# zoharl3/mantaflow

Measured on AMD Instinct MI355X. Metric: Mcells/s per step (advect+CG+FLIP), 256^3 grid, higher is better.
Workload: dtype f32; 1 GPU; 256^3 smoke step on 1 x MI355X: advectSemiLagrange(density, order 2) + advectSemiLagrange(vel, order 2) + setWallBcs + solvePressure (MIC-CG, cgAccuracy 1e-3); parallelism=single GPU

## Files before the change

### mantaflow_amd/csrc/pressure.hip

```cpp
#include "common.h"
#include "pressure.h"
#include <float.h>
#include <stdlib.h>
#include <stdio.h>
#include <type_traits>

using namespace mf;

static thread_local int g_last_shortcut[3] = {0, 0, 0};


__device__ __forceinline__ float wave_shr1(float v) {
	return __int_as_float(__builtin_amdgcn_update_dpp(__float_as_int(v), __float_as_int(v), 0x138, 0xf, 0xf, false));
}
__device__ __forceinline__ float wave_shl1(float v) {
	return __int_as_float(__builtin_amdgcn_update_dpp(__float_as_int(v), __float_as_int(v), 0x130, 0xf, 0xf, false));
}
__device__ __forceinline__ int4 unpack_flags(unsigned w) {
	return make_int4((w & 0x1u) ? MF_FLUID : 0, (w & 0x100u) ? MF_FLUID : 0, (w & 0x10000u) ? MF_FLUID : 0, (w & 0x1000000u) ? MF_FLUID : 0);
}
template <unsigned BIT>
__device__ __forceinline__ float4 unpack_coef(unsigned w) {
	return make_float4((w & BIT) ? -1.f : 0.f, (w & (BIT << 8)) ? -1.f : 0.f, (w & (BIT << 16)) ? -1.f : 0.f, (w & (BIT << 24)) ? -1.f : 0.f);
}
#ifndef AM_NT
#define AM_NT 2
#endif
#ifndef PCG_NT_MI
#define PCG_NT_MI 10
#endif
constexpr int64_t PCG_NT_CELLS = (int64_t)PCG_NT_MI << 20;
#ifndef AMP_NT
#define AMP_NT 1
#endif
template <bool DOT, bool IS3D, int R, bool PACKED>
__global__ void __launch_bounds__(BLOCK)
k_apply_matrix_v5(Dim d, const int32_t* __restrict__ flags, float* __restrict__ dst, const float* __restrict__ src,
                  const float* __restrict__ A0, const float* __restrict__ Ai, const float* __restrict__ Aj,
                  const float* __restrict__ Ak, double* __restrict__ partials, const CgScalars* __restrict__ sc, int jgroups, int tpb,
                  const unsigned char* __restrict__ pack, int dk0, int dk1, int a0p, const int* __restrict__ bempty = nullptr, int nbj = 0,
                  const int* __restrict__ outside_bad = nullptr, const int* __restrict__ xr = nullptr) {
	if (DOT && sc->done) return;
	const int qx = d.sx >> 2;
	const int64_t nthr = (int64_t)qx * jgroups * d.sz;
	const int vb0 = xcd_swizzle(blockIdx.x, gridDim.x) * tpb;
	double acc = 0.0;
#pragma unroll 1
	for (int t = 0; t < tpb; t++) {
	const int64_t T0 = (int64_t)(vb0 + t) * BLOCK + threadIdx.x;
	const bool live = T0 < nthr;
	const int64_t T = live ? T0 : nthr - 1;
	const int qi = (int)(T % qx);
	const int64_t rg = T / qx;
	const int j0 = (int)(rg % jgroups) * R;
	const int k = (int)(rg / jgroups);
	int q_lo = 0, q_hi = qx;
	if (IS3D && bempty && outside_bad[0] == 0) {
		if (xr) {
			q_lo = (xr[0] & ~7) >> 2;
			q_hi = ((xr[1] + 7) & ~7) >> 2;
		}
		if (bempty[(k >> 3) * nbj + (j0 >> 3)] || qi < q_lo || qi >= q_hi) continue;
	}
	const int lane = threadIdx.x & 63;
	const float4 z4 = make_float4(0.f, 0.f, 0.f, 0.f);
	const int64_t Y = d.Y, Z = d.Z;
	const int64_t row0 = ((int64_t)k * d.sy + j0) * d.sx + 4 * qi;
	int4 f[R];
	float4 sv[R + 2], ajv[R + 1], a0[R], ai[R], ak[R], akm[R], szm[R], szp[R];
	float sl[R], al[R], sr[R];
	{
		const int jm = (rg > 0) ? -1 : 0;
		sv[0] = *(const float4*)(src + row0 + jm * Y);
		if (PACKED) ajv[0] = unpack_coef<4u>(*(const unsigned*)(pack + row0 + jm * Y));
		else ajv[0] = *(const float4*)(Aj + row0 + jm * Y);
	}
#pragma unroll
	for (int r = 0; r < R; r++) {
		const int jr = (j0 + r < d.sy) ? r : (d.sy - 1 - j0);
		const int64_t idx = row0 + jr * Y;
		sv[r + 1] = ((AMP_NT & 1) && (!DOT || (a0p & 2))) ? ld_nt4(src + idx) : *(const float4*)(src + idx);
		unsigned pw = 0;
		if (PACKED) pw = *(const unsigned*)(pack + idx);
		if (PACKED && (a0p & 1)) a0[r] = make_float4((float)((pw >> 4) & 15u), (float)((pw >> 12) & 15u), (float)((pw >> 20) & 15u), (float)((pw >> 28) & 15u));
		else a0[r] = (AM_NT >= 1) ? ld_nt4(A0 + idx) : *(const float4*)(A0 + idx);
		if (PACKED) {
			f[r] = unpack_flags(pw);
			ajv[r + 1] = unpack_coef<4u>(pw);
			ai[r] = unpack_coef<2u>(pw);
		} else {
			f[r] = (AM_NT >= 1) ? ld_nt4i(flags + idx) : *(const int4*)(flags + idx);
			ajv[r + 1] = (AM_NT >= 3) ? ld_nt4(Aj + idx) : *(const float4*)(Aj + idx);
			ai[r] = (AM_NT >= 1) ? ld_nt4(Ai + idx) : *(const float4*)(Ai + idx);
		}
		if (IS3D) {
			const int64_t im = (k > 0) ? idx - Z : idx, ip = (k < d.sz - 1) ? idx + Z : idx;
			if (PACKED) {
				ak[r] = unpack_coef<8u>(pw);
				akm[r] = unpack_coef<8u>(*(const unsigned*)(pack + im));
			} else {
				ak[r] = (AM_NT >= 3) ? ld_nt4(Ak + idx) : *(const float4*)(Ak + idx);
				akm[r] = *(const float4*)(Ak + im);
			}
			szm[r] = (AMP_NT & 2) ? ld_nt4(src + im) : *(const float4*)(src + im);
			szp[r] = (AMP_NT & 2) ? ld_nt4(src + ip) : *(const float4*)(src + ip);
		}
	}
	{
		const int jr = (j0 + R < d.sy) ? R : (d.sy - j0 - ((k < d.sz - 1) ? 0 : 1));
		sv[R + 1] = *(const float4*)(src + row0 + jr * Y);
	}
	const bool edge_l = (lane == 0) || (qi == 0) || (qi == q_lo), edge_r = (lane == 63) || (qi == qx - 1) || (qi == q_hi - 1);
#pragma unroll
	for (int r = 0; r < R; r++) {
		const int jr = (j0 + r < d.sy) ? r : (d.sy - 1 - j0);
		const int64_t idx = row0 + jr * Y;
		sl[r] = wave_shr1(sv[r + 1].w);
		al[r] = wave_shr1(ai[r].w);
		sr[r] = wave_shl1(sv[r + 1].x);
		if (edge_l) {
			sl[r] = (idx > 0) ? src[idx - 1] : 0.f;
			if (PACKED) al[r] = (idx > 0 && (pack[idx - 1] & 2u)) ? -1.f : 0.f;
			else al[r] = (idx > 0) ? Ai[idx - 1] : 0.f;
		}
		if (edge_r) sr[r] = (idx + 4 < d.n) ? src[idx + 4] : 0.f;
	}
#pragma unroll
	for (int r = 0; r < R; r++) {
		const int j = j0 + r;
		if (j >= d.sy) break;
		const int4 fl = f[r];
		const float4 s = sv[r + 1];
		float4 res = s;
		if ((fl.x | fl.y | fl.z | fl.w) & MF_FLUID) {
			const float4 sym = (j > 0 || k > 0) ? sv[r] : z4, ajm = (j > 0 || k > 0) ? ajv[r] : z4;
			const float4 syp = (j < d.sy - 1) ? sv[r + 2] : (k < d.sz - 1) ? sv[R + 1] : z4, aj = ajv[r + 1];
			float4 zm = z4, am = z4, zp = z4, akc = z4;
			if (IS3D) {
				akc = ak[r];
				if (k > 0) {
					zm = szm[r];
					am = akm[r];
				}
				if (k < d.sz - 1) zp = szp[r];
			}
#define CELL5(c, SL, AL, SR)                                                                      \
	if (fl.c & MF_FLUID) {                                                                        \
		float v = s.c * a0[r].c;                                                                  \
		v = v + (SL) * (AL);                                                                      \
		v = v + (SR) * ai[r].c;                                                                   \
		v = v + sym.c * ajm.c;                                                                    \
		v = v + syp.c * aj.c;                                                                     \
		if (IS3D) {                                                                               \
			v = v + zm.c * am.c;                                                                  \
			v = v + zp.c * akc.c;                                                                 \
		}                                                                                         \
		res.c = v;                                                                                \
	}
			CELL5(x, sl[r], al[r], s.y)
			CELL5(y, s.x, ai[r].x, s.z)
			CELL5(z, s.y, ai[r].y, s.w)
			CELL5(w, s.z, ai[r].z, sr[r])
#undef CELL5
		}
		if (live) {
			if (AM_NT >= 2 && (!DOT || (a0p & 2))) st_nt4(dst + row0 + r * Y, res);
			else *(float4*)(dst + row0 + r * Y) = res;
			if (DOT && k >= dk0 && k < dk1) {
				const float p0 = res.x * s.x, p1 = res.y * s.y, p2 = res.z * s.z, p3 = res.w * s.w;
				acc += (double)p0;
				acc += (double)p1;
				acc += (double)p2;
				acc += (double)p3;
			}
		}
	}
	}
	if (DOT) {
		acc = block_sum(acc);
		if (threadIdx.x == 0) partials[blockIdx.x] = acc;
	}
}

template <bool DOT>
__global__ void __launch_bounds__(BLOCK)
k_apply_matrix_scalar(Dim d, const int32_t* __restrict__ flags, float* __restrict__ dst, const float* __restrict__ src,
                      const float* __restrict__ A0, const float* __restrict__ Ai, const float* __restrict__ Aj,
                      const float* __restrict__ Ak, double* __restrict__ partials, const CgScalars* __restrict__ sc) {
	if (DOT && sc->done) return;
	double acc = 0.0;
	for (int64_t idx = blockIdx.x * (int64_t)BLOCK + threadIdx.x; idx < d.n; idx += (int64_t)gridDim.x * BLOCK) {
		const float s = src[idx];
		float v = s;
		if (flags[idx] & MF_FLUID) {
			const int64_t Y = d.Y, Z = d.Z;
			v = s * A0[idx];
			v = v + ((idx >= 1) ? src[idx - 1] * Ai[idx - 1] : 0.f);
			v = v + ((idx + 1 < d.n) ? src[idx + 1] : 0.f) * Ai[idx];
			v = v + ((idx >= Y) ? src[idx - Y] * Aj[idx - Y] : 0.f);
			v = v + ((idx + Y < d.n) ? src[idx + Y] : 0.f) * Aj[idx];
			if (d.is3d) {
				v = v + ((idx >= Z) ? src[idx - Z] * Ak[idx - Z] : 0.f);
				v = v + ((idx + Z < d.n) ? src[idx + Z] : 0.f) * Ak[idx];
			}
		}
		dst[idx] = v;
		if (DOT) {
			const float p = v * s;
			acc += (double)p;
		}
	}
	if (DOT) {
		acc = block_sum(acc);
		if (threadIdx.x == 0) partials[blockIdx.x] = acc;
	}
}


struct AmOpts {
	const unsigned char* pack = nullptr;
	bool a0p = false;
	int dk0 = 0, dk1 = 0x7fffffff;
	const int* bempty = nullptr;
	int nbj = 0;
	const int* outside_bad = nullptr;
	const int* xr = nullptr;
	int nt = -1;
};
template <bool DOT>
static int launch_apply_matrix(const Dim& d, const int32_t* flags, float* dst, const float* src, const float* A0,
                               const float* Ai, const float* Aj, const float* Ak, double* partials,
                               const CgScalars* sc, hipStream_t st, const AmOpts& o = AmOpts{}, int* nblocks = nullptr, bool* ranged = nullptr) {
	if (ranged) *ranged = false;
	const int a0pn = (o.a0p ? 1 : 0) | ((DOT && (o.nt < 0 ? d.n > PCG_NT_CELLS : o.nt != 0)) ? 2 : 0);
	const bool vec = (d.sx % 4 == 0) && al16(flags) && al16(dst) && al16(src) && al16(A0) && al16(Ai) && al16(Aj) && al16(Ak);
	int nb;
	if (vec) {
		constexpr int R = 2;
		const int jgroups = (d.sy + R - 1) / R;
		const int64_t vblocks = ((int64_t)(d.sx >> 2) * jgroups * d.sz + BLOCK - 1) / BLOCK;
		const int tpb = (int)((vblocks + MAX_BLOCKS - 1) / MAX_BLOCKS);
		nb = (int)((vblocks + tpb - 1) / tpb);
		auto kern = !d.is3d ? k_apply_matrix_v5<DOT, false, R, false> : o.pack ? k_apply_matrix_v5<DOT, true, R, true> : k_apply_matrix_v5<DOT, true, R, false>;
		hipLaunchKernelGGL(kern, dim3(nb), dim3(BLOCK), 0, st, d, flags, dst, src, A0, Ai, Aj, Ak, partials, sc, jgroups, tpb, o.pack, o.dk0, o.dk1, a0pn,
		                   o.bempty, o.nbj, o.outside_bad, o.xr);
		if (ranged) *ranged = true;
	} else {
		nb = blocks_for(d.n, BLOCK, 2048);
		hipLaunchKernelGGL((k_apply_matrix_scalar<DOT>), dim3(nb), dim3(BLOCK), 0, st, d, flags, dst, src, A0, Ai, Aj, Ak, partials, sc);
	}
	MF_LAUNCH_CHECK();
	if (nblocks) *nblocks = nb;
	return 0;
}

__global__ void __launch_bounds__(BLOCK)
k_make_laplace(Dim d, const int32_t* __restrict__ flags, float* __restrict__ A0, float* __restrict__ Ai,
               float* __restrict__ Aj, float* __restrict__ Ak, const float* __restrict__ fr) {
	CELL_IJK(d)
	if (!INTERIOR(d)) return;
	if (!(flags[idx] & MF_FLUID)) return;
	const int64_t Y = d.Y, Z = d.Z;
	float a0 = A0[idx];
	if (!fr) {
		if (!(flags[idx - 1] & MF_OBSTACLE)) a0 = (float)((double)a0 + 1.);
		if (!(flags[idx + 1] & MF_OBSTACLE)) a0 = (float)((double)a0 + 1.);
		if (!(flags[idx - Y] & MF_OBSTACLE)) a0 = (float)((double)a0 + 1.);
		if (!(flags[idx + Y] & MF_OBSTACLE)) a0 = (float)((double)a0 + 1.);
		if (d.is3d && !(flags[idx - Z] & MF_OBSTACLE)) a0 = (float)((double)a0 + 1.);
		if (d.is3d && !(flags[idx + Z] & MF_OBSTACLE)) a0 = (float)((double)a0 + 1.);
		if (flags[idx + 1] & MF_FLUID) Ai[idx] = -1.f;
		if (flags[idx + Y] & MF_FLUID) Aj[idx] = -1.f;
		if (d.is3d && (flags[idx + Z] & MF_FLUID)) Ak[idx] = -1.f;
	} else {
		const float *fx = fr, *fy = fr + d.n, *fz = fr + 2 * d.n;
		a0 += fx[idx];
		a0 += fx[idx + 1];
		a0 += fy[idx];
		a0 += fy[idx + Y];
		if (d.is3d) a0 += fz[idx];
		if (d.is3d) a0 += fz[idx + Z];
		if (flags[idx + 1] & MF_FLUID) Ai[idx] = -fx[idx + 1];
		if (flags[idx + Y] & MF_FLUID) Aj[idx] = -fy[idx + Y];
		if (d.is3d && (flags[idx + Z] & MF_FLUID)) Ak[idx] = -fz[idx + Z];
	}
	A0[idx] = a0;
}

__device__ __forceinline__ float thetaHelper(float inside, float outside) {
	const float denom = inside - outside;
	if ((double)denom > -1e-04) return 0.5f;
	const float q = inside / denom;
	const float m = q < 1.f ? q : 1.f;
	return 0.f < m ? m : 0.f;
}
__device__ __forceinline__ float ghostFluidHelper(int64_t idx, int64_t offset, const float* __restrict__ phi, float gfClamp) {
	const float alpha = thetaHelper(phi[idx], phi[idx + offset]);
	if (alpha < gfClamp) return gfClamp;
	return (float)(1. - (1. / (double)alpha));
}
__device__ __forceinline__ float surfTensHelper(int64_t idx, int64_t offset, const float* __restrict__ phi,
                                                const float* __restrict__ curv, float surfTens, float gfClamp) {
	return surfTens * (curv[idx + offset] - ghostFluidHelper(idx, offset, phi, gfClamp) * curv[idx]);
}
__device__ __forceinline__ bool ghostFluidWasClamped(int64_t idx, int64_t offset, const float* __restrict__ phi, float gfClamp) {
	return thetaHelper(phi[idx], phi[idx + offset]) < gfClamp;
}

__global__ void __launch_bounds__(BLOCK)
k_make_rhs(Dim d, const int32_t* __restrict__ flags, float* __restrict__ rhs, const float* __restrict__ vel,
           const float* __restrict__ pcc, const float* __restrict__ fr, const float* __restrict__ ob,
           const float* __restrict__ phi, const float* __restrict__ curv, float surfTens, float gfClamp,
           double* __restrict__ partials) {
	double mysum = 0.0, mycnt = 0.0;
	const int64_t X = 1, Y = d.Y, Z = d.Z, n = d.n;
	const float *vx = vel, *vy = vel + n, *vz = vel + 2 * n;
	for (int64_t idx = blockIdx.x * (int64_t)BLOCK + threadIdx.x; idx < n; idx += (int64_t)gridDim.x * BLOCK) {
		const int i = (int)(idx % d.sx);
		const int j = (int)((idx / d.sx) % d.sy);
		const int k = (int)(idx / ((int64_t)d.sx * d.sy));
		if (!INTERIOR(d)) continue;
		if (!(flags[idx] & MF_FLUID)) {
			rhs[idx] = 0.f;
			continue;
		}
		float set;
		if (!fr) {
			set = vx[idx] - vx[idx + X] + vy[idx] - vy[idx + Y];
			if (d.is3d) set += vz[idx] - vz[idx + Z];
		} else {
			const float *fx = fr, *fy = fr + n, *fz = fr + 2 * n;
			set = fx[idx] * vx[idx] - fx[idx + X] * vx[idx + X] + fy[idx] * vy[idx] - fy[idx + Y] * vy[idx + Y];
			if (d.is3d) set += fz[idx] * vz[idx] - fz[idx + Z] * vz[idx + Z];
			if (ob) {
				const float *ox = ob, *oy = ob + n, *oz = ob + 2 * n;
				set += (1 - fx[idx]) * ox[idx] - (1 - fx[idx + X]) * ox[idx + X] + (1 - fy[idx]) * oy[idx] -
				       (1 - fy[idx + Y]) * oy[idx + Y];
				if (d.is3d) set += (1 - fz[idx]) * oz[idx] - (1 - fz[idx + Z]) * oz[idx + Z];
			}
		}
		if (phi && curv) {
			if (flags[idx - X] & MF_EMPTY) set += surfTensHelper(idx, -X, phi, curv, surfTens, gfClamp);
			if (flags[idx + X] & MF_EMPTY) set += surfTensHelper(idx, +X, phi, curv, surfTens, gfClamp);
			if (flags[idx - Y] & MF_EMPTY) set += surfTensHelper(idx, -Y, phi, curv, surfTens, gfClamp);
			if (flags[idx + Y] & MF_EMPTY) set += surfTensHelper(idx, +Y, phi, curv, surfTens, gfClamp);
			if (d.is3d) {
				if (flags[idx - Z] & MF_EMPTY) set += surfTensHelper(idx, -Z, phi, curv, surfTens, gfClamp);
				if (flags[idx + Z] & MF_EMPTY) set += surfTensHelper(idx, +Z, phi, curv, surfTens, gfClamp);
			}
		}
		if (pcc) set += pcc[idx];
		mysum += (double)set;
		mycnt += 1.0;
		rhs[idx] = set;
	}
	mysum = block_sum(mysum);
	__syncthreads();
	mycnt = block_sum(mycnt);
	if (threadIdx.x == 0) {
		partials[blockIdx.x] = mysum;
		partials[MAX_BLOCKS + blockIdx.x] = mycnt;
	}
}
__global__ void __launch_bounds__(BLOCK) k_sum2_finish(int nb, const double* __restrict__ p0, const double* __restrict__ p1, double* __restrict__ out) {
	double a = strided_sum(p0, nb), b = strided_sum(p1, nb);
	a = block_sum(a);
	__syncthreads();
	b = block_sum(b);
	if (threadIdx.x == 0) {
		out[0] = a;
		out[1] = b;
	}
}

__global__ void __launch_bounds__(BLOCK)
k_ghost_fluid_diag(Dim d, float* __restrict__ A0, const int32_t* __restrict__ flags, const float* __restrict__ phi, float gfClamp) {
	CELL_IJK(d)
	if (!INTERIOR(d)) return;
	if (!(flags[idx] & MF_FLUID)) return;
	const int64_t X = 1, Y = d.Y, Z = d.Z;
	float a = A0[idx];
	if (flags[idx - X] & MF_EMPTY) a -= ghostFluidHelper(idx, -X, phi, gfClamp);
	if (flags[idx + X] & MF_EMPTY) a -= ghostFluidHelper(idx, +X, phi, gfClamp);
	if (flags[idx - Y] & MF_EMPTY) a -= ghostFluidHelper(idx, -Y, phi, gfClamp);
	if (flags[idx + Y] & MF_EMPTY) a -= ghostFluidHelper(idx, +Y, phi, gfClamp);
	if (d.is3d) {
		if (flags[idx - Z] & MF_EMPTY) a -= ghostFluidHelper(idx, -Z, phi, gfClamp);
		if (flags[idx + Z] & MF_EMPTY) a -= ghostFluidHelper(idx, +Z, phi, gfClamp);
	}
	A0[idx] = a;
}

__global__ void __launch_bounds__(BLOCK)
k_correct_velocity(Dim d, const int32_t* __restrict__ flags, float* __restrict__ vel, const float* __restrict__ p) {
	CELL_IJK(d)
	if (!INTERIOR(d)) return;
	const int64_t X = 1, Y = d.Y, Z = d.Z, n = d.n;
	float *vx = vel, *vy = vel + n, *vz = vel + 2 * n;
	const int f = flags[idx];
	if (f & MF_FLUID) {
		const float pc = p[idx];
		float x = vx[idx], y = vy[idx], z = d.is3d ? vz[idx] : 0.f;
		const int fxm = flags[idx - X], fym = flags[idx - Y], fzm = d.is3d ? flags[idx - Z] : 0;
		if (fxm & MF_FLUID) x -= (pc - p[idx - X]);
		if (fym & MF_FLUID) y -= (pc - p[idx - Y]);
		if (d.is3d && (fzm & MF_FLUID)) z -= (pc - p[idx - Z]);
		if (fxm & MF_EMPTY) x -= pc;
		if (fym & MF_EMPTY) y -= pc;
		if (d.is3d && (fzm & MF_EMPTY)) z -= pc;
		vx[idx] = x;
		vy[idx] = y;
		if (d.is3d) vz[idx] = z;
	} else if ((f & MF_EMPTY) && !(f & MF_OUTFLOW)) {
		if (flags[idx - X] & MF_FLUID) vx[idx] += p[idx - X]; else vx[idx] = 0.f;
		if (flags[idx - Y] & MF_FLUID) vy[idx] += p[idx - Y]; else vy[idx] = 0.f;
		if (d.is3d) {
			if (flags[idx - Z] & MF_FLUID) vz[idx] += p[idx - Z]; else vz[idx] = 0.f;
		}
	}
}

__global__ void __launch_bounds__(BLOCK)
k_correct_velocity_gf(Dim d, float* __restrict__ vel, const int32_t* __restrict__ flags, const float* __restrict__ p,
                      const float* __restrict__ phi, float gfClamp, const float* __restrict__ curv, float surfTens) {
	CELL_IJK(d)
	if (!INTERIOR(d)) return;
	const int64_t X = 1, Y = d.Y, Z = d.Z, n = d.n;
	float *vx = vel, *vy = vel + n, *vz = vel + 2 * n;
	const int f = flags[idx];
	const bool fl = (f & MF_FLUID) != 0, emp = (f & MF_EMPTY) && !(f & MF_OUTFLOW);
	if (fl) {
		if (flags[idx - X] & MF_EMPTY) vx[idx] += p[idx] * ghostFluidHelper(idx, -X, phi, gfClamp);
		if (flags[idx - Y] & MF_EMPTY) vy[idx] += p[idx] * ghostFluidHelper(idx, -Y, phi, gfClamp);
		if (d.is3d && (flags[idx - Z] & MF_EMPTY)) vz[idx] += p[idx] * ghostFluidHelper(idx, -Z, phi, gfClamp);
	} else if (emp) {
		if (flags[idx - X] & MF_FLUID) vx[idx] -= p[idx - X] * ghostFluidHelper(idx - X, +X, phi, gfClamp); else vx[idx] = 0.f;
		if (flags[idx - Y] & MF_FLUID) vy[idx] -= p[idx - Y] * ghostFluidHelper(idx - Y, +Y, phi, gfClamp); else vy[idx] = 0.f;
		if (d.is3d) {
			if (flags[idx - Z] & MF_FLUID) vz[idx] -= p[idx - Z] * ghostFluidHelper(idx - Z, +Z, phi, gfClamp); else vz[idx] = 0.f;
		}
	}
	if (curv) {
		if (fl) {
			if (flags[idx - X] & MF_EMPTY) vx[idx] += surfTensHelper(idx, -X, phi, curv, surfTens, gfClamp);
			if (flags[idx - Y] & MF_EMPTY) vy[idx] += surfTensHelper(idx, -Y, phi, curv, surfTens, gfClamp);
			if (d.is3d && (flags[idx - Z] & MF_EMPTY)) vz[idx] += surfTensHelper(idx, -Z, phi, curv, surfTens, gfClamp);
		} else if (emp) {
			vx[idx] -= (flags[idx - X] & MF_FLUID) ? surfTensHelper(idx - X, +X, phi, curv, surfTens, gfClamp) : 0.f;
			vy[idx] -= (flags[idx - Y] & MF_FLUID) ? surfTensHelper(idx - Y, +Y, phi, curv, surfTens, gfClamp) : 0.f;
			if (d.is3d) vz[idx] -= (flags[idx - Z] & MF_FLUID) ? surfTensHelper(idx - Z, +Z, phi, curv, surfTens, gfClamp) : 0.f;
		}
	}
}

__global__ void __launch_bounds__(BLOCK)
k_replace_clamped_gf(Dim d, float* __restrict__ vel, const int32_t* __restrict__ flags, const float* __restrict__ phi, float gfClamp) {
	CELL_IJK(d)
	if (!INTERIOR(d)) return;
	if (!(flags[idx] & MF_EMPTY)) return;
	const int64_t X = 1, Y = d.Y, Z = d.Z, n = d.n;
	float *vx = vel, *vy = vel + n, *vz = vel + 2 * n;
	if ((flags[idx - X] & MF_FLUID) && ghostFluidWasClamped(idx - X, +X, phi, gfClamp)) vx[idx] = vx[idx - X];
	if ((flags[idx - Y] & MF_FLUID) && ghostFluidWasClamped(idx - Y, +Y, phi, gfClamp)) vy[idx] = vy[idx - Y];
	if (d.is3d && (flags[idx - Z] & MF_FLUID) && ghostFluidWasClamped(idx - Z, +Z, phi, gfClamp)) vz[idx] = vz[idx - Z];
	if ((flags[idx + X] & MF_FLUID) && ghostFluidWasClamped(idx + X, -X, phi, gfClamp)) vx[idx] = vx[idx + X];
	if ((flags[idx + Y] & MF_FLUID) && ghostFluidWasClamped(idx + Y, -Y, phi, gfClamp)) vy[idx] = vy[idx + Y];
	if (d.is3d && (flags[idx + Z] & MF_FLUID) && ghostFluidWasClamped(idx + Z, -Z, phi, gfClamp)) vz[idx] = vz[idx + Z];
}

__global__ void k_fix_pressure(Dim d, int64_t p, float value, float* rhs, float* A0, float* Ai, float* Aj, float* Ak) {
	const int64_t X = 1, Y = d.Y, Z = d.Z;
	rhs[p + X] -= Ai[p] * value;
	rhs[p + Y] -= Aj[p] * value;
	rhs[p - X] -= Ai[p - X] * value;
	rhs[p - Y] -= Aj[p - Y] * value;
	if (d.is3d) {
		rhs[p + Z] -= Ak[p] * value;
		rhs[p - Z] -= Ak[p - Z] * value;
	}
	rhs[p] = value;
	A0[p] = 1.f;
	Ai[p] = Aj[p] = Ak[p] = 0.f;
	Ai[p - X] = 0.f;
	Aj[p - Y] = 0.f;
	if (d.is3d) Ak[p - Z] = 0.f;
}

__global__ void __launch_bounds__(BLOCK) k_cg_begin(CgScalars* sc, int nb, const double* __restrict__ partials, float accuracy, int useL2) {
	double acc = strided_sum(partials, nb);
	acc = block_sum(acc);
	if (threadIdx.x == 0) {
		sc->sigma = (float)acc;
		sc->alpha = sc->nalpha = sc->beta = 0.f;
		sc->resNorm = 1e20f;
		sc->accuracy = accuracy;
		sc->iterations = 0;
		sc->done = 0;
		sc->diverged = 0;
		sc->useL2 = useL2;
	}
}
__global__ void __launch_bounds__(BLOCK) k_cg_alpha(CgScalars* sc, int nb, const double* __restrict__ partials) {
	if (sc->done) {
		if (threadIdx.x == 0) sc->xpending = 0;
		return;
	}
	if (sc->diverged) {
		if (threadIdx.x == 0) {
			sc->done = 1;
			sc->xpending = 0;
		}
		return;
	}
	double acc = strided_sum(partials, nb);
	acc = block_sum(acc);
	if (threadIdx.x == 0) {
		const float dp = (float)acc;
		float alpha = 0.f;
		if (fabs((double)dp) > 0.) alpha = sc->sigma / dp;
		sc->dp = dp;
		sc->alpha = alpha;
		sc->nalpha = -alpha;
		sc->iterations++;
		sc->xpending = 1;
	}
}
template <bool COPY_TMP, bool EDOT = false>
__global__ void __launch_bounds__(BLOCK)
k_cg_axpy_r(int64_t n, const CgScalars* __restrict__ sc, float* __restrict__ residual, float* __restrict__ tmp, float* __restrict__ fpart,
            double* __restrict__ dpart, const int* __restrict__ bempty = nullptr, int nbj = 0, int sx = 0, int sy = 0,
            double* __restrict__ epart = nullptr, const int* __restrict__ outside_bad = nullptr, const int* __restrict__ xr = nullptr, int nt = 0) {
	if (sc->done) return;
	const bool zero_outside = EDOT && outside_bad[0] == 0;
	const int xlo = (EDOT && xr) ? (xr[0] & ~7) : 0, xhi = (EDOT && xr) ? ((xr[1] + 7) & ~7) : 0x7fffffff;
	const float nalpha = sc->nalpha;
	const bool l2 = sc->useL2 != 0;
	float lo = FLT_MAX, hi = -FLT_MAX;
	double ss = 0.0, es = 0.0;
	const int64_t n4 = n >> 2;
	for (int64_t q = blockIdx.x * (int64_t)BLOCK + threadIdx.x; q < n4; q += (int64_t)gridDim.x * BLOCK) {
// ... 1017 lines not shown
```

Measured before the change: 237.3 Mcells/s.

## Add z-marching apply-matrix kernel reusing neighbor rows in registers

```diff
diff --git a/mantaflow_amd/csrc/pressure.hip b/mantaflow_amd/csrc/pressure.hip
--- a/mantaflow_amd/csrc/pressure.hip
+++ b/mantaflow_amd/csrc/pressure.hip
@@ -182,6 +182,188 @@
 	}
 }
 
+#ifndef ZM_L
+#define ZM_L 16
+#endif
+#ifndef ZM_R
+#define ZM_R 2
+#endif
+constexpr int ZM_MAX_BLOCKS = 512;
+template <int R>
+struct ZmRest {
+	float4 ym, yp;
+	unsigned pw[R], pwm;
+	float sl[R], sr[R];
+	unsigned pl[R];
+};
+template <bool NT, int R>
+__device__ __forceinline__ void zm_load_rows(float4 (&s)[R], const Dim& d, const float* __restrict__ src, int64_t row0, int j0) {
+#pragma unroll
+	for (int r = 0; r < R; r++) {
+		const int jr = (j0 + r < d.sy) ? r : (d.sy - 1 - j0);
+		s[r] = NT ? ld_nt4(src + row0 + jr * d.Y) : *(const float4*)(src + row0 + jr * d.Y);
+	}
+}
+template <bool A0S, int R>
+__device__ __forceinline__ void zm_load_rest(ZmRest<R>& p, float4 (&a0)[R], const Dim& d, const float* __restrict__ src, const float* __restrict__ A0,
+                                             const unsigned char* __restrict__ pack, int64_t row0, int j0, int k) {
+	const int64_t Y = d.Y;
+	const int jm = (k > 0 || j0 > 0) ? -1 : 0;
+	const int jp = (j0 + R < d.sy) ? R : (d.sy - j0 - ((k < d.sz - 1) ? 0 : 1));
+	p.ym = *(const float4*)(src + row0 + jm * Y);
+	p.pwm = *(const unsigned*)(pack + row0 + jm * Y);
+	p.yp = *(const float4*)(src + row0 + jp * Y);
+#pragma unroll
+	for (int r = 0; r < R; r++) {
+		const int jr = (j0 + r < d.sy) ? r : (d.sy - 1 - j0);
+		const int64_t idx = row0 + jr * Y;
+		p.pw[r] = *(const unsigned*)(pack + idx);
+		if (A0S) a0[r] = (AM_NT >= 1) ? ld_nt4(A0 + idx) : *(const float4*)(A0 + idx);
+		const int64_t il = (idx > 0) ? idx - 1 : 0, ir = (idx + 4 < d.n) ? idx + 4 : idx;
+		p.sl[r] = src[il];
+		p.pl[r] = (unsigned)pack[il];
+		p.sr[r] = src[ir];
+	}
+}
+template <int R>
+__device__ __forceinline__ void zm_fix_rest(ZmRest<R>& p, const Dim& d, int64_t row0, int j0, int k) {
+	const float4 z4 = make_float4(0.f, 0.f, 0.f, 0.f);
+	if (!(k > 0 || j0 > 0)) {
+		p.ym = z4;
+		p.pwm = 0u;
+	}
+	if (!(k < d.sz - 1 || j0 + R < d.sy)) p.yp = z4;
+#pragma unroll
+	for (int r = 0; r < R; r++) {
+		const int jr = (j0 + r < d.sy) ? r : (d.sy - 1 - j0);
+		const int64_t idx = row0 + jr * d.Y;
+		if (!(idx > 0)) {
+			p.sl[r] = 0.f;
+			p.pl[r] = 0u;
+		}
+		if (!(idx + 4 < d.n)) p.sr[r] = 0.f;
+	}
+}
+template <bool DOT, bool A0S, bool NT>
+__global__ void __launch_bounds__(BLOCK)
+k_apply_matrix_zmarch(Dim d, float* __restrict__ dst, const float* __restrict__ src, const float* __restrict__ A0,
+                      const unsigned char* __restrict__ pack, double* __restrict__ partials, const CgScalars* __restrict__ sc, int jgroups,
+                      int tpb) {
+	constexpr int R = ZM_R, L = ZM_L;
+	if (DOT && sc->done) return;
+	const unsigned qx = (unsigned)(d.sx >> 2);
+	const unsigned per_seg = qx * (unsigned)jgroups;
+	const unsigned nthr = per_seg * (unsigned)((d.sz + L - 1) / L);
+	const int vb0 = xcd_swizzle(blockIdx.x, gridDim.x) * tpb;
+	const int lane = threadIdx.x & 63;
+	const float4 z4 = make_float4(0.f, 0.f, 0.f, 0.f);
+	const int64_t Y = d.Y, Z = d.Z;
+	double acc = 0.0;
+#pragma unroll 1
+	for (int t = 0; t < tpb; t++) {
+		const unsigned T0 = (unsigned)(vb0 + t) * BLOCK + threadIdx.x;
+		if (T0 >= nthr) continue;
+		const unsigned T = T0;
+		const unsigned seg = T / per_seg, in_seg = T - seg * per_seg;
+		const unsigned jg = in_seg / qx;
+		const int qi = (int)(in_seg - jg * qx), j0 = (int)jg * R;
+		const int k0 = (int)seg * L, k1 = (k0 + L < d.sz) ? k0 + L : d.sz;
+		const bool edge_l = (lane == 0) || (qi == 0), edge_r = (lane == 63) || (qi == (int)qx - 1);
+		const int64_t row00 = ((int64_t)k0 * d.sy + j0) * d.sx + 4 * qi;
+
+		auto step = [&](int k, const float4 (&sm)[R], const float4 (&s0)[R], const float4 (&s1)[R], float4 (&s2)[R], ZmRest<R>& c,
+		                ZmRest<R>& n, const float4 (&a0c)[R], float4 (&a0n)[R], const float4 (&akm)[R], float4 (&ako)[R]) __attribute__((always_inline)) {
+			const int64_t row0 = row00 + (int64_t)(k - k0) * Z;
+			const int kn = (k + 1 < d.sz) ? k + 1 : d.sz - 1, k2 = (k + 2 < d.sz) ? k + 2 : d.sz - 1;
+			zm_load_rest<A0S, R>(n, a0n, d, src, A0, pack, row00 + (int64_t)(kn - k0) * Z, j0, kn);
+			zm_load_rows<NT, R>(s2, d, src, row00 + (int64_t)(k2 - k0) * Z, j0);
+			zm_fix_rest<R>(c, d, row0, j0, k);
+			const bool top = k == d.sz - 1;
+			float4 aj[R + 1], res[R];
+			aj[0] = unpack_coef<4u>(c.pwm);
+#pragma unroll
+			for (int r = 0; r < R; r++) {
+				const unsigned pw = c.pw[r];
+				const float4 s = s0[r], ai = unpack_coef<2u>(pw), akc = unpack_coef<8u>(pw);
+				aj[r + 1] = unpack_coef<4u>(pw);
+				ako[r] = akc;
+				float sl = wave_shr1(s.w), sr = wave_shl1(s.x);
+				float al = (__float_as_uint(wave_shr1(__uint_as_float(pw))) & 0x02000000u) ? -1.f : 0.f;
+				if (edge_l) {
+					sl = c.sl[r];
+					al = (c.pl[r] & 2u) ? -1.f : 0.f;
+				}
+				if (edge_r) sr = c.sr[r];
+				const float4 a0 = A0S ? a0c[r] : make_float4((float)((pw >> 4) & 15u), (float)((pw >> 12) & 15u), (float)((pw >> 20) & 15u), (float)((pw >> 28) & 15u));
+				const float4 sym = (r == 0) ? c.ym : s0[r > 0 ? r - 1 : 0], ajm = aj[r];
+				const float4 syp = (r + 1 < R) ? ((j0 + r < d.sy - 1) ? s0[r + 1 < R ? r + 1 : 0] : c.yp) : c.yp, ajc = aj[r + 1];
+				const float4 zm = sm[r], am = akm[r], zp = top ? z4 : s1[r];
+#define CELL5(c_, BYTE, SL, AL, SR)                                                                   \
+	{                                                                                             \
+		float v = s.c_ * a0.c_;                                                                   \
+		v = v + (SL) * (AL);                                                                      \
+		v = v + (SR) * ai.c_;                                                                     \
+		v = v + sym.c_ * ajm.c_;                                                                  \
+		v = v + syp.c_ * ajc.c_;                                                                  \
+		v = v + zm.c_ * am.c_;                                                                    \
+		v = v + zp.c_ * akc.c_;                                                                   \
+		res[r].c_ = (pw & (1u << (8 * BYTE))) ? v : s.c_;                                         \
+	}
+				CELL5(x, 0, sl, al, s.y)
+				CELL5(y, 1, s.x, ai.x, s.z)
+				CELL5(z, 2, s.y, ai.y, s.w)
+				CELL5(w, 3, s.z, ai.z, sr)
+#undef CELL5
+				if (DOT && j0 + r < d.sy) {
+					const float p0 = res[r].x * s.x, p1 = res[r].y * s.y, p2 = res[r].z * s.z, p3 = res[r].w * s.w;
+					acc += (double)p0;
+					acc += (double)p1;
+					acc += (double)p2;
+					acc += (double)p3;
+				}
+			}
+#pragma unroll
+			for (int r = 0; r < R; r++) {
+				const bool own = j0 + r < d.sy;
+				const float4 o = own ? res[r] : res[0];
+				float* const p = dst + row0 + (own ? r : 0) * Y;
+				if (AM_NT >= 2 && NT) st_nt4(p, o);
+				else *(float4*)p = o;
+			}
+		};
+
+		float4 sa[R], sb[R], sc_[R], sd[R], a0a[R], a0b[R], aka[R], akb[R];
+		ZmRest<R> ca, cb;
+#pragma unroll
+		for (int r = 0; r < R; r++) sa[r] = aka[r] = z4;
+		zm_load_rows<NT, R>(sb, d, src, row00, j0);
+		zm_load_rest<A0S, R>(ca, a0a, d, src, A0, pack, row00, j0, k0);
+		zm_load_rows<NT, R>(sc_, d, src, row00 + ((k0 + 1 < d.sz) ? Z : 0), j0);
+		if (k0 > 0) {
+			zm_load_rows<false, R>(sa, d, src, row00 - Z, j0);
+#pragma unroll
+			for (int r = 0; r < R; r++) {
+				const int jr = (j0 + r < d.sy) ? r : (d.sy - 1 - j0);
+				aka[r] = unpack_coef<8u>(*(const unsigned*)(pack + row00 - Z + jr * Y));
+			}
+		}
+#pragma unroll 1
+		for (int k = k0; k < k1; k += 4) {
+			step(k, sa, sb, sc_, sd, ca, cb, a0a, a0b, aka, akb);
+			if (k + 1 >= k1) break;
+			step(k + 1, sb, sc_, sd, sa, cb, ca, a0b, a0a, akb, aka);
+			if (k + 2 >= k1) break;
+			step(k + 2, sc_, sd, sa, sb, ca, cb, a0a, a0b, aka, akb);
+			if (k + 3 >= k1) break;
+			step(k + 3, sd, sa, sb, sc_, cb, ca, a0b, a0a, akb, aka);
+		}
+	}
+	if (DOT) {
+		acc = block_sum(acc);
+		if (threadIdx.x == 0) partials[blockIdx.x] = acc;
+	}
+}
+
 template <bool DOT>
 __global__ void __launch_bounds__(BLOCK)
 k_apply_matrix_scalar(Dim d, const int32_t* __restrict__ flags, float* __restrict__ dst, const float* __restrict__ src,
@@ -235,7 +417,17 @@
 	const int a0pn = (o.a0p ? 1 : 0) | ((DOT && (o.nt < 0 ? d.n > PCG_NT_CELLS : o.nt != 0)) ? 2 : 0);
 	const bool vec = (d.sx % 4 == 0) && al16(flags) && al16(dst) && al16(src) && al16(A0) && al16(Ai) && al16(Aj) && al16(Ak);
 	int nb;
-	if (vec) {
+	if (vec && d.is3d && o.pack && !o.bempty && o.dk0 <= 0 && o.dk1 >= d.sz) {
+		const int jgroups = (d.sy + ZM_R - 1) / ZM_R;
+		const int64_t vblocks = ((int64_t)(d.sx >> 2) * jgroups * ((d.sz + ZM_L - 1) / ZM_L) + BLOCK - 1) / BLOCK;
+		const int tpb = (int)((vblocks + ZM_MAX_BLOCKS - 1) / ZM_MAX_BLOCKS);
+		nb = (int)((vblocks + tpb - 1) / tpb);
+		const bool a0s = !(a0pn & 1), nt = !DOT || (a0pn & 2);
+		auto kern = nt ? (a0s ? k_apply_matrix_zmarch<DOT, true, true> : k_apply_matrix_zmarch<DOT, false, true>)
+		               : (a0s ? k_apply_matrix_zmarch<DOT, true, !DOT> : k_apply_matrix_zmarch<DOT, false, !DOT>);
+		hipLaunchKernelGGL(kern, dim3(nb), dim3(BLOCK), 0, st, d, dst, src, A0, o.pack, partials, sc, jgroups, tpb);
+		if (ranged) *ranged = true;
+	} else if (vec) {
 		constexpr int R = 2;
 		const int jgroups = (d.sy + R - 1) / R;
 		const int64_t vblocks = ((int64_t)(d.sx >> 2) * jgroups * d.sz + BLOCK - 1) / BLOCK;
```

After: 243.1 Mcells/s (median of 6 runs). 1.02x the previous value.
